# frutiemax92/YAT

Measured on AMD Instinct MI355X. Metric: images/sec (whole node) SANA-1.6B 1024px bf16 training step, higher is better.
Workload: dtype bf16; 1 GPU; train_sana.py: SANA-1.6B (D=2240, 20 blocks) 1024px, bf16, full fine-tune, cached latents/text embeds, aspect buckets [(32, 32), (16, 64), (24, 42), (44, 22)] round-robin, prompts of 20..300 tokens (text rows packed: the masked padding rows to T=512 are not computed), AdamW+clip; global_batch=8, per_gpu_batch=8, seq_len=1024, parallelism=dp1, num_layers=20, params=1604462784

## Files before the change

### yat_amd/csrc/linear_attn.hip

```cpp
#include "common.hpp"
#include "../../include/yat_hip.h"

namespace {

constexpr int C = 32;
constexpr int SS = 33 * C;
constexpr int TB = 256;

__device__ __forceinline__ bf16x8 zero8() {
    bf16x8 z;
#pragma unroll
    for (int e = 0; e < 8; ++e) z[e] = (__bf16)0.0f;
    return z;
}
__device__ __forceinline__ bf16x8 relu8(bf16x8 v) {
    u32x4 u = __builtin_bit_cast(u32x4, v);
#pragma unroll
    for (int i = 0; i < 4; ++i) {
        const uint32_t neg = (u[i] >> 15) & 0x00010001u;
        u[i] &= ~(neg * 0xffffu);
    }
    return __builtin_bit_cast(bf16x8, u);
}
__device__ __forceinline__ void split8(const float* x, bf16x8& hi, bf16x8& lo) {
#pragma unroll
    for (int e = 0; e < 8; ++e) {
        const __bf16 h = (__bf16)x[e];
        hi[e] = h;
        lo[e] = (__bf16)(x[e] - (float)h);
    }
}
__device__ __forceinline__ void state_frag_rows(const float* S, int row0, int nrows, int lane, bf16x8& hi, bf16x8& lo) {
    float x[8];
    const int r = row0 + (lane & 15);
    if (r < nrows) {
        const f32x4 a = *reinterpret_cast<const f32x4*>(S + r * C + 8 * (lane >> 4));
        const f32x4 b = *reinterpret_cast<const f32x4*>(S + r * C + 8 * (lane >> 4) + 4);
        x[0] = a[0]; x[1] = a[1]; x[2] = a[2]; x[3] = a[3]; x[4] = b[0]; x[5] = b[1]; x[6] = b[2]; x[7] = b[3];
    } else {
#pragma unroll
        for (int e = 0; e < 8; ++e) x[e] = 0.f;
    }
    split8(x, hi, lo);
}
template <bool ACC_ORDER>
__device__ __forceinline__ void state_frag_cols(const float* S, int col0, int lane, bf16x8& hi, bf16x8& lo) {
    float x[8];
    const int c = col0 + (lane & 15), g = lane >> 4;
#pragma unroll
    for (int j = 0; j < 8; ++j) {
        const int cp = ACC_ORDER ? (j < 4 ? 4 * g + j : 16 + 4 * g + (j - 4)) : 8 * g + j;
        x[j] = S[cp * C + c];
    }
    split8(x, hi, lo);
}
__device__ __forceinline__ void acc2frag_hilo(const f32x4& a, const f32x4& b, bf16x8& hi, bf16x8& lo) {
    const float x[8] = {a[0], a[1], a[2], a[3], b[0], b[1], b[2], b[3]};
    split8(x, hi, lo);
}
__device__ __forceinline__ bf16x8 tok_frag(const bf16_t* base, int ld, int tok, int N, int lane) {
    bf16x8 z = zero8();
    if (tok < N) z = *reinterpret_cast<const bf16x8*>(base + (int64_t)tok * ld + 8 * (lane >> 4));
    return z;
}
__device__ __forceinline__ u32x2 tok4_raw(const bf16_t* base, int ld, int tok, int N, int c0) {
    return tok < N ? *reinterpret_cast<const u32x2*>(base + (int64_t)tok * ld + c0) : u32x2{0u, 0u};
}
__device__ __forceinline__ void tok4(const bf16_t* base, int ld, int tok, int N, int c0, float* o) {
    if (tok < N) unpack4(*reinterpret_cast<const u32x2*>(base + (int64_t)tok * ld + c0), o);
    else { o[0] = o[1] = o[2] = o[3] = 0.f; }
}

__global__ __launch_bounds__(256) void la_state_kernel(int N, const bf16_t* qkv, int ld, int k_off, int v_off,
                                                       uint64_t bytes, float* S_out) {
    __shared__ __attribute__((aligned(16))) char lds[4 * 8192 + 4 * 6 * 64 * 16];
    const int lane = threadIdx.x & 63, wave = __builtin_amdgcn_readfirstlane(threadIdx.x >> 6);
    int h, b, unused_z;
    xcd_contiguous3(h, b, unused_z);
    char* kt = lds + wave * 8192;
    char* vt = kt + 4096;
    const __amdgpu_buffer_rsrc_t rs = make_rsrc(qkv, bytes);
    const int per = ((N + 3) / 4 + 63) / 64 * 64;
    const int n_begin = wave * per, n_end = min(N, n_begin + per);
    const int64_t head_off = (int64_t)b * N * ld + h * C;

    f32x4 acc[2][3];
#pragma unroll
    for (int i = 0; i < 2; ++i)
#pragma unroll
        for (int j = 0; j < 3; ++j) acc[i][j] = f32x4{0.f, 0.f, 0.f, 0.f};
    bf16x8 ones = zero8();
    if ((lane & 15) == 0) {
#pragma unroll
        for (int e = 0; e < 8; ++e) ones[e] = (__bf16)1.0f;
    }
    const uint32_t g = lane >> 4, q4 = (lane & 15) >> 2, p4 = lane & 3;
    for (int n0 = n_begin; n0 < n_end; n0 += 64) {
#pragma unroll
        for (int pc = 0; pc < 4; ++pc) {
            const int r = pc * 16 + (lane >> 2);
            const int slot = lane & 3;
            const int chunk = slot ^ (((r >> 3) & 1) << 1);
            const int n = n0 + r;
            const uint32_t vk = n < N ? (uint32_t)((head_off + (int64_t)n * ld + k_off + chunk * 8) * 2) : YAT_OOB;
            const uint32_t vv = n < N ? (uint32_t)((head_off + (int64_t)n * ld + v_off + chunk * 8) * 2) : YAT_OOB;
            lds_dma16(rs, (YAT_LDS void*)(kt + pc * 1024), vk);
            lds_dma16(rs, (YAT_LDS void*)(vt + pc * 1024), vv);
        }
        asm volatile("s_waitcnt vmcnt(0)" ::: "memory");
#pragma unroll
        for (int ks = 0; ks < 2; ++ks) {
            bf16x8 kf[2], vf[2];
#pragma unroll
            for (int ct = 0; ct < 2; ++ct) {
                const uint32_t col = ct * 16 + 4 * p4;
                const uint32_t r0 = ks * 32 + 8 * g + q4, r1 = r0 + 4;
                const uint32_t c0 = (col >> 3) ^ (((r0 >> 3) & 1) << 1), c1 = (col >> 3) ^ (((r1 >> 3) & 1) << 1);
                kf[ct] = relu8(cat4(lds_read_tr4(kt, r0 * 64 + c0 * 16 + (p4 & 1) * 8), lds_read_tr4(kt, r1 * 64 + c1 * 16 + (p4 & 1) * 8)));
                vf[ct] = cat4(lds_read_tr4(vt, r0 * 64 + c0 * 16 + (p4 & 1) * 8), lds_read_tr4(vt, r1 * 64 + c1 * 16 + (p4 & 1) * 8));
            }
#pragma unroll
            for (int ct = 0; ct < 2; ++ct) {
                acc[ct][0] = mfma16(kf[ct], vf[0], acc[ct][0]);
                acc[ct][1] = mfma16(kf[ct], vf[1], acc[ct][1]);
                acc[ct][2] = mfma16(kf[ct], ones, acc[ct][2]);
            }
        }
        asm volatile("s_waitcnt lgkmcnt(0)" ::: "memory");
    }
    float* red = reinterpret_cast<float*>(lds + 4 * 8192);
#pragma unroll
    for (int ct = 0; ct < 2; ++ct)
#pragma unroll
        for (int j = 0; j < 3; ++j) *reinterpret_cast<f32x4*>(red + ((wave * 6 + ct * 3 + j) * 64 + lane) * 4) = acc[ct][j];
    __syncthreads();
    if (wave == 0) {
        float* S = S_out + ((int64_t)b * gridDim.x + h) * SS;
#pragma unroll
        for (int ct = 0; ct < 2; ++ct)
#pragma unroll
            for (int j = 0; j < 3; ++j) {
                f32x4 s = f32x4{0.f, 0.f, 0.f, 0.f};
#pragma unroll
                for (int w = 0; w < 4; ++w) {
                    const f32x4 t = *reinterpret_cast<const f32x4*>(red + ((w * 6 + ct * 3 + j) * 64 + lane) * 4);
                    s[0] += t[0]; s[1] += t[1]; s[2] += t[2]; s[3] += t[3];
                }
                const int cp = j * 16 + (lane & 15);
                if (cp < 33) {
#pragma unroll
                    for (int r = 0; r < 4; ++r) S[cp * C + ct * 16 + 4 * g + r] = s[r];
                }
            }
    }
}

__device__ __forceinline__ void u_tiles(const bf16x8 (&shi)[3], const bf16x8 (&slo)[3], bf16x8 qf, f32x4 (&ut)[3]) {
#pragma unroll
    for (int t = 0; t < 3; ++t) {
        ut[t] = mfma16(shi[t], qf, f32x4{0.f, 0.f, 0.f, 0.f});
        ut[t] = mfma16(slo[t], qf, ut[t]);
    }
}

__global__ __launch_bounds__(256) void la_fwd_kernel(int N, int H, const bf16_t* qkv, int ld, const float* S_all,
                                                     bf16_t* out, int ld_out) {
    const int lane = threadIdx.x & 63, wave = threadIdx.x >> 6;
    int cx, h, b;
    xcd_contiguous3(cx, h, b);
    const float* S = S_all + ((int64_t)b * H + h) * SS;
    bf16x8 shi[3], slo[3];
#pragma unroll
    for (int t = 0; t < 3; ++t) state_frag_rows(S, t * 16, 33, lane, shi[t], slo[t]);
    const bf16_t* qb = qkv + (int64_t)b * N * ld + h * C;
    bf16_t* ob = out + (int64_t)b * N * ld_out + h * C;
    const int g = lane >> 4, li = lane & 15;
    bf16x8 qfr[4];
#pragma unroll
    for (int grp = 0; grp < 4; ++grp) qfr[grp] = tok_frag(qb, ld, cx * TB + wave * 64 + grp * 16 + li, N, lane);
#pragma unroll
    for (int grp = 0; grp < 4; ++grp) {
        const int n = cx * TB + wave * 64 + grp * 16 + li;
        f32x4 ut[3];
        u_tiles(shi, slo, relu8(qfr[grp]), ut);
        const float den = __shfl(ut[2][0], li, 64) + 1e-15f;
        const float inv = 1.0f / den;
        if (n < N) {
#pragma unroll
            for (int t = 0; t < 2; ++t)
                *reinterpret_cast<u32x2*>(ob + (int64_t)n * ld_out + t * 16 + 4 * g) =
                    pack4(ut[t][0] * inv, ut[t][1] * inv, ut[t][2] * inv, ut[t][3] * inv);
        }
    }
}

__device__ __forceinline__ uint32_t du_off(uint32_t row, uint32_t byte) {
    const uint32_t sw = (((row >> 1) & 1) | (((row >> 3) & 1) << 1)) << 1;
    return row * 128 + ((((byte >> 4) ^ sw) << 4) | (byte & 15));
}
__device__ __forceinline__ uint32_t q_off(uint32_t row, uint32_t byte) {
    return row * 64 + (byte ^ (((row >> 3) & 1) << 5));
}

__global__ __launch_bounds__(256, 3) void la_bwd_q_kernel(int N, int H, const bf16_t* qkv, int ld, const bf16_t* dout, int ld_do,
                                                       const float* S_all, bf16_t* dqkv, int ld_dq, float* dS_part) {
    __shared__ __attribute__((aligned(16))) char lds[4 * (2 * 4096 + 2048)];
    static_assert(4 * 6 * 64 * 16 <= 4 * (2 * 4096 + 2048), "reduction slab must fit in the images");
    const int lane = threadIdx.x & 63, wave = __builtin_amdgcn_readfirstlane(threadIdx.x >> 6);
    int cx, h, b;
    xcd_contiguous3(cx, h, b);
    const int g = lane >> 4, li = lane & 15, q4 = li >> 2, p4 = lane & 3;
    const float* S = S_all + ((int64_t)b * H + h) * SS;
    char* du_img = lds + wave * 10240;
    char* du_lo = du_img + 4096;
    char* q_img = du_img + 8192;
    bf16x8 shi[3], slo[3], xhi[2], xlo[2];
#pragma unroll
    for (int t = 0; t < 3; ++t) state_frag_rows(S, t * 16, 33, lane, shi[t], slo[t]);
#pragma unroll
    for (int ct = 0; ct < 2; ++ct) state_frag_cols<true>(S, ct * 16, lane, xhi[ct], xlo[ct]);
    float s32[2][4];
#pragma unroll
    for (int ct = 0; ct < 2; ++ct)
#pragma unroll
        for (int r = 0; r < 4; ++r) s32[ct][r] = S[32 * C + ct * 16 + 4 * g + r];
    const bf16_t* qb = qkv + (int64_t)b * N * ld + h * C;
    const bf16_t* dob = dout + (int64_t)b * N * ld_do + h * C;
    bf16_t* dqb = dqkv + (int64_t)b * N * ld_dq + h * C;

    f32x4 ds[3][2];
#pragma unroll
    for (int t = 0; t < 3; ++t)
#pragma unroll
        for (int ct = 0; ct < 2; ++ct) ds[t][ct] = f32x4{0.f, 0.f, 0.f, 0.f};

    bf16x8 qfr[4];
    u32x2 d4r[4][2], q4r[4][2];
#pragma unroll
    for (int s4 = 0; s4 < 4; ++s4) {
        const int n = cx * TB + wave * 64 + s4 * 16 + li;
        qfr[s4] = tok_frag(qb, ld, n, N, lane);
#pragma unroll
        for (int t = 0; t < 2; ++t) {
            d4r[s4][t] = tok4_raw(dob, ld_do, n, N, t * 16 + 4 * g);
            q4r[s4][t] = tok4_raw(qb, ld, n, N, t * 16 + 4 * g);
        }
    }
#pragma unroll
    for (int half = 0; half < 2; ++half) {
#pragma unroll
        for (int sub = 0; sub < 2; ++sub) {
            const int n0 = cx * TB + wave * 64 + half * 32 + sub * 16;
            const int n = n0 + li;
            const bf16x8 qf = relu8(qfr[half * 2 + sub]);
            f32x4 ut[3];
            u_tiles(shi, slo, qf, ut);
            const float den = __shfl(ut[2][0], li, 64) + 1e-15f;
            const float inv = 1.0f / den;
            float dot = 0.f;
            f32x4 du[2];
#pragma unroll
            for (int t = 0; t < 2; ++t) {
                float d4[4];
                unpack4(d4r[half * 2 + sub][t], d4);
#pragma unroll
                for (int r = 0; r < 4; ++r) {
                    dot += d4[r] * (ut[t][r] * inv);
                    du[t][r] = d4[r] * inv;
                }
            }
            dot += __shfl_xor(dot, 16, 64);
            dot += __shfl_xor(dot, 32, 64);
            const float du32 = -dot * inv;
            bf16x8 dhi, dlo;
            acc2frag_hilo(du[0], du[1], dhi, dlo);
            const bool valid = n < N;
#pragma unroll
            for (int ct = 0; ct < 2; ++ct) {
                f32x4 dq = mfma16(xhi[ct], dhi, f32x4{0.f, 0.f, 0.f, 0.f});
                dq = mfma16(xhi[ct], dlo, dq);
                dq = mfma16(xlo[ct], dhi, dq);
                float q4v[4];
                unpack4(q4r[half * 2 + sub][ct], q4v);
                if (valid) {
                    float o[4];
#pragma unroll
                    for (int r = 0; r < 4; ++r) o[r] = q4v[r] > 0.f ? dq[r] + s32[ct][r] * du32 : 0.f;
                    *reinterpret_cast<u32x2*>(dqb + (int64_t)n * ld_dq + ct * 16 + 4 * g) = pack4(o[0], o[1], o[2], o[3]);
                }
            }
            const int trow = sub * 16 + li;
#pragma unroll
            for (int t = 0; t < 2; ++t) {
                float hi4[4], lo4[4];
#pragma unroll
                for (int r = 0; r < 4; ++r) { hi4[r] = valid ? rbf(du[t][r]) : 0.f; lo4[r] = valid ? du[t][r] - hi4[r] : 0.f; }
                *reinterpret_cast<u32x2*>(du_img + du_off(trow, (t * 16 + 4 * g) * 2)) = pack4(hi4[0], hi4[1], hi4[2], hi4[3]);
                *reinterpret_cast<u32x2*>(du_lo + du_off(trow, (t * 16 + 4 * g) * 2)) = pack4(lo4[0], lo4[1], lo4[2], lo4[3]);
            }
            {
                const float h32 = (valid && g == 0) ? rbf(du32) : 0.f, l32 = (valid && g == 0) ? du32 - h32 : 0.f;
                *reinterpret_cast<u32x2*>(du_img + du_off(trow, (32 + 4 * g) * 2)) = pack4(h32, 0.f, 0.f, 0.f);
                *reinterpret_cast<u32x2*>(du_lo + du_off(trow, (32 + 4 * g) * 2)) = pack4(l32, 0.f, 0.f, 0.f);
            }
            *reinterpret_cast<u32x2*>(du_img + du_off(trow, (48 + 4 * g) * 2)) = u32x2{0u, 0u};
            *reinterpret_cast<u32x2*>(du_lo + du_off(trow, (48 + 4 * g) * 2)) = u32x2{0u, 0u};
            *reinterpret_cast<bf16x8*>(q_img + q_off(trow, g * 16)) = qf;
        }
        asm volatile("s_waitcnt lgkmcnt(0)" ::: "memory");
        bf16x8 af[3], al[3], bfr[2];
        const uint32_t r0 = 8 * g + q4, r1 = r0 + 4;
#pragma unroll
        for (int t = 0; t < 3; ++t) {
            const uint32_t off = (t * 16 + 4 * p4) * 2;
            af[t] = cat4(lds_read_tr4(du_img, du_off(r0, off)), lds_read_tr4(du_img, du_off(r1, off)));
            al[t] = cat4(lds_read_tr4(du_lo, du_off(r0, off)), lds_read_tr4(du_lo, du_off(r1, off)));
        }
#pragma unroll
        for (int ct = 0; ct < 2; ++ct) {
            const uint32_t off = (ct * 16 + 4 * p4) * 2;
            bfr[ct] = cat4(lds_read_tr4(q_img, q_off(r0, off)), lds_read_tr4(q_img, q_off(r1, off)));
        }
#pragma unroll
        for (int t = 0; t < 3; ++t)
#pragma unroll
            for (int ct = 0; ct < 2; ++ct) {
                ds[t][ct] = mfma16(af[t], bfr[ct], ds[t][ct]);
                ds[t][ct] = mfma16(al[t], bfr[ct], ds[t][ct]);
            }
        asm volatile("s_waitcnt lgkmcnt(0)" ::: "memory");
    }
    __syncthreads();
    float* red = reinterpret_cast<float*>(lds);
#pragma unroll
    for (int t = 0; t < 3; ++t)
#pragma unroll
        for (int ct = 0; ct < 2; ++ct) *reinterpret_cast<f32x4*>(red + ((wave * 6 + t * 2 + ct) * 64 + lane) * 4) = ds[t][ct];
    __syncthreads();
    if (wave == 0) {
        float* slab = dS_part + (((int64_t)b * H + h) * gridDim.x + cx) * SS;
#pragma unroll
        for (int t = 0; t < 3; ++t)
#pragma unroll
            for (int ct = 0; ct < 2; ++ct) {
                f32x4 s = f32x4{0.f, 0.f, 0.f, 0.f};
#pragma unroll
                for (int w = 0; w < 4; ++w) {
                    const f32x4 v = *reinterpret_cast<const f32x4*>(red + ((w * 6 + t * 2 + ct) * 64 + lane) * 4);
                    s[0] += v[0]; s[1] += v[1]; s[2] += v[2]; s[3] += v[3];
                }
#pragma unroll
                for (int r = 0; r < 4; ++r) {
                    const int cp = t * 16 + 4 * g + r;
                    if (cp < 33) slab[cp * C + ct * 16 + li] = s[r];
                }
            }
    }
}

__global__ void la_reduce_slabs_kernel(int nbh, int nchunks, const float* part, float* dS) {
    const int64_t i = (int64_t)blockIdx.x * blockDim.x + threadIdx.x;
    if (i >= (int64_t)nbh * SS) return;
    const int64_t bh = i / SS, e = i % SS;
    float s = 0.f;
    for (int c = 0; c < nchunks; ++c) s += part[(bh * nchunks + c) * SS + e];
    dS[i] = s;
}

__global__ __launch_bounds__(256) void la_bwd_kv_kernel(int N, int H, const bf16_t* qkv, int ld, int k_off, int v_off,
                                                        const float* dS_all, bf16_t* dqkv, int ld_dq) {
    const int lane = threadIdx.x & 63, wave = threadIdx.x >> 6;
    int cx, h, b;
    xcd_contiguous3(cx, h, b);
    const int g = lane >> 4, li = lane & 15;
    const float* dS = dS_all + ((int64_t)b * H + h) * SS;
    bf16x8 rhi[2], rlo[2], chi[2], clo[2];
#pragma unroll
    for (int t = 0; t < 2; ++t) state_frag_rows(dS, t * 16, 32, lane, rhi[t], rlo[t]);
#pragma unroll
    for (int ct = 0; ct < 2; ++ct) state_frag_cols<false>(dS, ct * 16, lane, chi[ct], clo[ct]);
    float s32[2][4];
#pragma unroll
    for (int ct = 0; ct < 2; ++ct)
#pragma unroll
        for (int r = 0; r < 4; ++r) s32[ct][r] = dS[32 * C + ct * 16 + 4 * g + r];
    const bf16_t* kb = qkv + (int64_t)b * N * ld + h * C + k_off;
    const bf16_t* vb = qkv + (int64_t)b * N * ld + h * C + v_off;
    bf16_t* dkb = dqkv + (int64_t)b * N * ld_dq + h * C + k_off;
    bf16_t* dvb = dqkv + (int64_t)b * N * ld_dq + h * C + v_off;
    bf16x8 kfr[4], vfr[4];
    u32x2 k4r[4][2];
#pragma unroll
    for (int grp = 0; grp < 4; ++grp) {
        const int n = cx * TB + wave * 64 + grp * 16 + li;
        kfr[grp] = tok_frag(kb, ld, n, N, lane);
        vfr[grp] = tok_frag(vb, ld, n, N, lane);
#pragma unroll
        for (int t = 0; t < 2; ++t) k4r[grp][t] = tok4_raw(kb, ld, n, N, t * 16 + 4 * g);
    }
#pragma unroll
    for (int grp = 0; grp < 4; ++grp) {
        const int n = cx * TB + wave * 64 + grp * 16 + li;
        const bf16x8 kf = relu8(kfr[grp]);
        const bf16x8 vf = vfr[grp];
#pragma unroll
        for (int t = 0; t < 2; ++t) {
            f32x4 dv = mfma16(rhi[t], kf, f32x4{0.f, 0.f, 0.f, 0.f});
            dv = mfma16(rlo[t], kf, dv);
            f32x4 dk = mfma16(chi[t], vf, f32x4{0.f, 0.f, 0.f, 0.f});
            dk = mfma16(clo[t], vf, dk);
            float k4[4];
            unpack4(k4r[grp][t], k4);
            if (n < N) {
                *reinterpret_cast<u32x2*>(dvb + (int64_t)n * ld_dq + t * 16 + 4 * g) = pack4(dv[0], dv[1], dv[2], dv[3]);
                float o[4];
#pragma unroll
                for (int r = 0; r < 4; ++r) o[r] = k4[r] > 0.f ? dk[r] + s32[t][r] : 0.f;
                *reinterpret_cast<u32x2*>(dkb + (int64_t)n * ld_dq + t * 16 + 4 * g) = pack4(o[0], o[1], o[2], o[3]);
            }
        }
    }
}

}

extern "C" {

uint64_t yat_linear_attn_workspace_bytes(int B, int N, int H) {
    const uint64_t nchunks = (N + TB - 1) / TB;
    return (uint64_t)B * H * SS * sizeof(float) * (2 + nchunks);
}

static int la_check(int B, int N, int H, int ld, int k_off, int v_off) {
    if (B <= 0 || N <= 0 || H <= 0 || (ld & 7) || (k_off & 7) || (v_off & 7)) return YAT_EINVAL;
    if ((uint64_t)B * N * ld * 2 > 0x7fffffffull) return YAT_EINVAL;
    return YAT_OK;
}

int yat_linear_attn_fwd(int B, int N, int H, const void* qkv, int ld, int k_off, int v_off, void* out, int ld_out,
                        void* workspace, yat_stream_t stream) {
    if (la_check(B, N, H, ld, k_off, v_off) || (ld_out & 7) || !qkv || !out || !workspace) return YAT_EINVAL;
    float* S = (float*)workspace;
    hipLaunchKernelGGL(la_state_kernel, dim3(H, B), dim3(256), 0, (hipStream_t)stream, N, (const bf16_t*)qkv, ld, k_off, v_off,
                       (uint64_t)B * N * ld * 2, S);
    YAT_CHECK_LAUNCH();
    hipLaunchKernelGGL(la_fwd_kernel, dim3((N + TB - 1) / TB, H, B), dim3(256), 0, (hipStream_t)stream, N, H,
                       (const bf16_t*)qkv, ld, (const float*)S, (bf16_t*)out, ld_out);
    YAT_CHECK_LAUNCH();
    return YAT_OK;
}

int yat_linear_attn_bwd(int B, int N, int H, const void* qkv, int ld, int k_off, int v_off, const void* dout, int ld_dout,
                        void* dqkv, int ld_dqkv, const float* state, void* workspace, yat_stream_t stream) {
    if (la_check(B, N, H, ld, k_off, v_off) || (ld_dout & 7) || (ld_dqkv & 7) || !qkv || !dout || !dqkv || !workspace)
        return YAT_EINVAL;
    const int nchunks = (N + TB - 1) / TB;
    float* S = (float*)workspace;
    float* dS = S + (int64_t)B * H * SS;
    float* part = dS + (int64_t)B * H * SS;
    hipStream_t st = (hipStream_t)stream;
    if (state) {
        S = const_cast<float*>(state);
    } else {
        hipLaunchKernelGGL(la_state_kernel, dim3(H, B), dim3(256), 0, st, N, (const bf16_t*)qkv, ld, k_off, v_off,
                           (uint64_t)B * N * ld * 2, S);
        YAT_CHECK_LAUNCH();
    }
    hipLaunchKernelGGL(la_bwd_q_kernel, dim3(nchunks, H, B), dim3(256), 0, st, N, H, (const bf16_t*)qkv, ld,
                       (const bf16_t*)dout, ld_dout, (const float*)S, (bf16_t*)dqkv, ld_dqkv, part);
    YAT_CHECK_LAUNCH();
    const int64_t tot = (int64_t)B * H * SS;
    hipLaunchKernelGGL(la_reduce_slabs_kernel, dim3((unsigned)((tot + 255) / 256)), dim3(256), 0, st, B * H, nchunks,
                       (const float*)part, dS);
    YAT_CHECK_LAUNCH();
    hipLaunchKernelGGL(la_bwd_kv_kernel, dim3(nchunks, H, B), dim3(256), 0, st, N, H, (const bf16_t*)qkv, ld, k_off, v_off,
                       (const float*)dS, (bf16_t*)dqkv, ld_dqkv);
    YAT_CHECK_LAUNCH();
    return YAT_OK;
}

}
```

Before: 106.0 images/s.

## Fuse slab reduction into linear-attn bwd kv and pair heads for full-line stores

```diff
diff --git a/yat_amd/csrc/linear_attn.hip b/yat_amd/csrc/linear_attn.hip
--- a/yat_amd/csrc/linear_attn.hip
+++ b/yat_amd/csrc/linear_attn.hip
@@ -30,12 +30,35 @@
         lo[e] = (__bf16)(x[e] - (float)h);
     }
 }
-__device__ __forceinline__ void state_frag_rows(const float* S, int row0, int nrows, int lane, bf16x8& hi, bf16x8& lo) {
+struct OneState {
+    const float* S;
+    __device__ __forceinline__ float at(int i) const { return S[i]; }
+    __device__ __forceinline__ f32x4 at4(int i) const { return *reinterpret_cast<const f32x4*>(S + i); }
+};
+struct SlabSum {
+    const float* part;
+    int n;
+    __device__ __forceinline__ float at(int i) const {
+        float s = 0.f;
+        for (int c = 0; c < n; ++c) s += part[(int64_t)c * SS + i];
+        return s;
+    }
+    __device__ __forceinline__ f32x4 at4(int i) const {
+        f32x4 s = f32x4{0.f, 0.f, 0.f, 0.f};
+        for (int c = 0; c < n; ++c) {
+            const f32x4 t = *reinterpret_cast<const f32x4*>(part + (int64_t)c * SS + i);
+            s[0] += t[0]; s[1] += t[1]; s[2] += t[2]; s[3] += t[3];
+        }
+        return s;
+    }
+};
+template <class St>
+__device__ __forceinline__ void state_frag_rows(const St S, int row0, int nrows, int lane, bf16x8& hi, bf16x8& lo) {
     float x[8];
     const int r = row0 + (lane & 15);
     if (r < nrows) {
-        const f32x4 a = *reinterpret_cast<const f32x4*>(S + r * C + 8 * (lane >> 4));
-        const f32x4 b = *reinterpret_cast<const f32x4*>(S + r * C + 8 * (lane >> 4) + 4);
+        const f32x4 a = S.at4(r * C + 8 * (lane >> 4));
+        const f32x4 b = S.at4(r * C + 8 * (lane >> 4) + 4);
         x[0] = a[0]; x[1] = a[1]; x[2] = a[2]; x[3] = a[3]; x[4] = b[0]; x[5] = b[1]; x[6] = b[2]; x[7] = b[3];
     } else {
 #pragma unroll
@@ -43,14 +66,14 @@
     }
     split8(x, hi, lo);
 }
-template <bool ACC_ORDER>
-__device__ __forceinline__ void state_frag_cols(const float* S, int col0, int lane, bf16x8& hi, bf16x8& lo) {
+template <bool ACC_ORDER, class St>
+__device__ __forceinline__ void state_frag_cols(const St S, int col0, int lane, bf16x8& hi, bf16x8& lo) {
     float x[8];
     const int c = col0 + (lane & 15), g = lane >> 4;
 #pragma unroll
     for (int j = 0; j < 8; ++j) {
         const int cp = ACC_ORDER ? (j < 4 ? 4 * g + j : 16 + 4 * g + (j - 4)) : 8 * g + j;
-        x[j] = S[cp * C + c];
+        x[j] = S.at(cp * C + c);
     }
     split8(x, hi, lo);
 }
@@ -163,12 +186,13 @@
     }
 }
 
-__global__ __launch_bounds__(256) void la_fwd_kernel(int N, int H, const bf16_t* qkv, int ld, const float* S_all,
+__global__ __launch_bounds__(256) void la_fwd_kernel(int N, int H, int h0, const bf16_t* qkv, int ld, const float* S_all,
                                                      bf16_t* out, int ld_out) {
     const int lane = threadIdx.x & 63, wave = threadIdx.x >> 6;
     int cx, h, b;
     xcd_contiguous3(cx, h, b);
-    const float* S = S_all + ((int64_t)b * H + h) * SS;
+    h += h0;
+    const OneState S{S_all + ((int64_t)b * H + h) * SS};
     bf16x8 shi[3], slo[3];
 #pragma unroll
     for (int t = 0; t < 3; ++t) state_frag_rows(S, t * 16, 33, lane, shi[t], slo[t]);
@@ -192,6 +216,63 @@
                     pack4(ut[t][0] * inv, ut[t][1] * inv, ut[t][2] * inv, ut[t][3] * inv);
         }
     }
+}
+
+__device__ __forceinline__ uint32_t pair_off(uint32_t row, uint32_t byte) {
+    return row * 128 + ((swz128(row, byte >> 4) << 4) | (byte & 15));
+}
+__device__ __forceinline__ void pair_store_rows(const char* img, int rows, bf16_t* dst, int ld, int n0, int N, int lane) {
+    for (int r0 = 0; r0 < rows; r0 += 8) {
+        const int r = r0 + (lane >> 3), ch = lane & 7;
+        if (n0 + r < N)
+            *reinterpret_cast<u32x4*>(dst + (int64_t)(n0 + r) * ld + ch * 8) = *reinterpret_cast<const u32x4*>(img + pair_off(r, ch * 16));
+    }
+}
+__device__ __forceinline__ uint32_t pos_mask8(bf16x8 v) {
+    uint32_t m = 0;
+#pragma unroll
+    for (int e = 0; e < 8; ++e) m |= ((float)v[e] > 0.f ? 1u : 0u) << e;
+    return m;
+}
+__device__ __forceinline__ uint32_t out_layout_mask(uint32_t m8, int li, int g) {
+    const uint32_t lo = (uint32_t)__shfl((int)m8, li + 16 * (g >> 1), 64), hi = (uint32_t)__shfl((int)m8, li + 16 * (2 + (g >> 1)), 64);
+    const int sh = 4 * (g & 1);
+    return ((lo >> sh) & 15u) | (((hi >> sh) & 15u) << 4);
+}
+
+__global__ __launch_bounds__(256) void la_fwd_pair_kernel(int N, int H, const bf16_t* qkv, int ld, const float* S_all,
+                                                          bf16_t* out, int ld_out) {
+    __shared__ __attribute__((aligned(16))) char lds[4 * 8192];
+    const int lane = threadIdx.x & 63, wave = __builtin_amdgcn_readfirstlane(threadIdx.x >> 6);
+    int cx, hp, b;
+    xcd_contiguous3(cx, hp, b);
+    const int h = 2 * hp, g = lane >> 4, li = lane & 15, n0 = cx * TB + wave * 64;
+    char* img = lds + wave * 8192;
+    const bf16_t* qb = qkv + (int64_t)b * N * ld + h * C;
+    bf16x8 qfr[2][4];
+#pragma unroll
+    for (int grp = 0; grp < 4; ++grp)
+#pragma unroll
+        for (int hh = 0; hh < 2; ++hh) qfr[hh][grp] = tok_frag(qb + hh * C, ld, n0 + grp * 16 + li, N, lane);
+#pragma unroll
+    for (int hh = 0; hh < 2; ++hh) {
+        const OneState S{S_all + ((int64_t)b * H + h + hh) * SS};
+        bf16x8 shi[3], slo[3];
+#pragma unroll
+        for (int t = 0; t < 3; ++t) state_frag_rows(S, t * 16, 33, lane, shi[t], slo[t]);
+#pragma unroll
+        for (int grp = 0; grp < 4; ++grp) {
+            f32x4 ut[3];
+            u_tiles(shi, slo, relu8(qfr[hh][grp]), ut);
+            const float den = __shfl(ut[2][0], li, 64) + 1e-15f;
+            const float inv = 1.0f / den;
+#pragma unroll
+            for (int t = 0; t < 2; ++t)
+                *reinterpret_cast<u32x2*>(img + pair_off(grp * 16 + li, hh * 64 + t * 32 + 8 * g)) =
+                    pack4(ut[t][0] * inv, ut[t][1] * inv, ut[t][2] * inv, ut[t][3] * inv);
+        }
+    }
+    pair_store_rows(img, 64, out + (int64_t)b * N * ld_out + h * C, ld_out, n0, N, lane);
 }
 
 __device__ __forceinline__ uint32_t du_off(uint32_t row, uint32_t byte) {
@@ -216,9 +297,9 @@
     char* q_img = du_img + 8192;
     bf16x8 shi[3], slo[3], xhi[2], xlo[2];
 #pragma unroll
-    for (int t = 0; t < 3; ++t) state_frag_rows(S, t * 16, 33, lane, shi[t], slo[t]);
-#pragma unroll
-    for (int ct = 0; ct < 2; ++ct) state_frag_cols<true>(S, ct * 16, lane, xhi[ct], xlo[ct]);
+    for (int t = 0; t < 3; ++t) state_frag_rows(OneState{S}, t * 16, 33, lane, shi[t], slo[t]);
+#pragma unroll
+    for (int ct = 0; ct < 2; ++ct) state_frag_cols<true>(OneState{S}, ct * 16, lane, xhi[ct], xlo[ct]);
     float s32[2][4];
 #pragma unroll
     for (int ct = 0; ct < 2; ++ct)
@@ -358,67 +439,118 @@
     }
 }
 
-__global__ void la_reduce_slabs_kernel(int nbh, int nchunks, const float* part, float* dS) {
-    const int64_t i = (int64_t)blockIdx.x * blockDim.x + threadIdx.x;
-    if (i >= (int64_t)nbh * SS) return;
-    const int64_t bh = i / SS, e = i % SS;
-    float s = 0.f;
-    for (int c = 0; c < nchunks; ++c) s += part[(bh * nchunks + c) * SS + e];
-    dS[i] = s;
-}
-
-__global__ __launch_bounds__(256) void la_bwd_kv_kernel(int N, int H, const bf16_t* qkv, int ld, int k_off, int v_off,
-                                                        const float* dS_all, bf16_t* dqkv, int ld_dq) {
+struct KvState {
+    bf16x8 rhi[2], rlo[2], chi[2], clo[2];
+    float s32[2][4];
+    __device__ __forceinline__ void load(const SlabSum dS, int lane) {
+#pragma unroll
+        for (int t = 0; t < 2; ++t) state_frag_rows(dS, t * 16, 32, lane, rhi[t], rlo[t]);
+#pragma unroll
+        for (int ct = 0; ct < 2; ++ct) state_frag_cols<false>(dS, ct * 16, lane, chi[ct], clo[ct]);
+#pragma unroll
+        for (int ct = 0; ct < 2; ++ct) {
+            const f32x4 v = dS.at4(32 * C + ct * 16 + 4 * (lane >> 4));
+            s32[ct][0] = v[0]; s32[ct][1] = v[1]; s32[ct][2] = v[2]; s32[ct][3] = v[3];
+        }
+    }
+    __device__ __forceinline__ void apply(bf16x8 kraw, bf16x8 vf, uint32_t kpos, u32x2 (&dk2)[2], u32x2 (&dv2)[2]) const {
+        const bf16x8 kf = relu8(kraw);
+#pragma unroll
+        for (int t = 0; t < 2; ++t) {
+            f32x4 dv = mfma16(rhi[t], kf, f32x4{0.f, 0.f, 0.f, 0.f});
+            dv = mfma16(rlo[t], kf, dv);
+            f32x4 dk = mfma16(chi[t], vf, f32x4{0.f, 0.f, 0.f, 0.f});
+            dk = mfma16(clo[t], vf, dk);
+            float o[4];
+#pragma unroll
+            for (int r = 0; r < 4; ++r) o[r] = ((kpos >> (4 * t + r)) & 1u) ? dk[r] + s32[t][r] : 0.f;
+            dv2[t] = pack4(dv[0], dv[1], dv[2], dv[3]);
+            dk2[t] = pack4(o[0], o[1], o[2], o[3]);
+        }
+    }
+};
+
+__global__ __launch_bounds__(256) void la_bwd_kv_kernel(int N, int H, int h0, const bf16_t* qkv, int ld, int k_off, int v_off,
+                                                        const float* part, bf16_t* dqkv, int ld_dq) {
     const int lane = threadIdx.x & 63, wave = threadIdx.x >> 6;
     int cx, h, b;
     xcd_contiguous3(cx, h, b);
+    h += h0;
     const int g = lane >> 4, li = lane & 15;
-    const float* dS = dS_all + ((int64_t)b * H + h) * SS;
-    bf16x8 rhi[2], rlo[2], chi[2], clo[2];
-#pragma unroll
-    for (int t = 0; t < 2; ++t) state_frag_rows(dS, t * 16, 32, lane, rhi[t], rlo[t]);
-#pragma unroll
-    for (int ct = 0; ct < 2; ++ct) state_frag_cols<false>(dS, ct * 16, lane, chi[ct], clo[ct]);
-    float s32[2][4];
-#pragma unroll
-    for (int ct = 0; ct < 2; ++ct)
-#pragma unroll
-        for (int r = 0; r < 4; ++r) s32[ct][r] = dS[32 * C + ct * 16 + 4 * g + r];
     const bf16_t* kb = qkv + (int64_t)b * N * ld + h * C + k_off;
     const bf16_t* vb = qkv + (int64_t)b * N * ld + h * C + v_off;
     bf16_t* dkb = dqkv + (int64_t)b * N * ld_dq + h * C + k_off;
     bf16_t* dvb = dqkv + (int64_t)b * N * ld_dq + h * C + v_off;
     bf16x8 kfr[4], vfr[4];
-    u32x2 k4r[4][2];
 #pragma unroll
     for (int grp = 0; grp < 4; ++grp) {
         const int n = cx * TB + wave * 64 + grp * 16 + li;
         kfr[grp] = tok_frag(kb, ld, n, N, lane);
         vfr[grp] = tok_frag(vb, ld, n, N, lane);
-#pragma unroll
-        for (int t = 0; t < 2; ++t) k4r[grp][t] = tok4_raw(kb, ld, n, N, t * 16 + 4 * g);
-    }
+    }
+    KvState st;
+    st.load(SlabSum{part + ((int64_t)b * H + h) * gridDim.x * SS, (int)gridDim.x}, lane);
 #pragma unroll
     for (int grp = 0; grp < 4; ++grp) {
         const int n = cx * TB + wave * 64 + grp * 16 + li;
-        const bf16x8 kf = relu8(kfr[grp]);
-        const bf16x8 vf = vfr[grp];
-#pragma unroll
-        for (int t = 0; t < 2; ++t) {
-            f32x4 dv = mfma16(rhi[t], kf, f32x4{0.f, 0.f, 0.f, 0.f});
-            dv = mfma16(rlo[t], kf, dv);
-            f32x4 dk = mfma16(chi[t], vf, f32x4{0.f, 0.f, 0.f, 0.f});
-            dk = mfma16(clo[t], vf, dk);
-            float k4[4];
-            unpack4(k4r[grp][t], k4);
-            if (n < N) {
-                *reinterpret_cast<u32x2*>(dvb + (int64_t)n * ld_dq + t * 16 + 4 * g) = pack4(dv[0], dv[1], dv[2], dv[3]);
-                float o[4];
-#pragma unroll
-                for (int r = 0; r < 4; ++r) o[r] = k4[r] > 0.f ? dk[r] + s32[t][r] : 0.f;
-                *reinterpret_cast<u32x2*>(dkb + (int64_t)n * ld_dq + t * 16 + 4 * g) = pack4(o[0], o[1], o[2], o[3]);
-            }
-        }
+        u32x2 dk2[2], dv2[2];
+        st.apply(kfr[grp], vfr[grp], out_layout_mask(pos_mask8(kfr[grp]), li, g), dk2, dv2);
+        if (n < N) {
+#pragma unroll
+            for (int t = 0; t < 2; ++t) {
+                *reinterpret_cast<u32x2*>(dvb + (int64_t)n * ld_dq + t * 16 + 4 * g) = dv2[t];
+                *reinterpret_cast<u32x2*>(dkb + (int64_t)n * ld_dq + t * 16 + 4 * g) = dk2[t];
+            }
+        }
+    }
+}
+
+constexpr int KV_ST = 16;
+__global__ __launch_bounds__(256) void la_bwd_kv_pair_kernel(int N, int H, const bf16_t* qkv, int ld, int k_off, int v_off,
+                                                             const float* part, bf16_t* dqkv, int ld_dq) {
+    constexpr int SUB = KV_ST / 16, IMG = KV_ST * 128;
+    __shared__ __attribute__((aligned(16))) char lds[2 * 2 * 2 * IMG];
+    const int lane = threadIdx.x & 63, wave = __builtin_amdgcn_readfirstlane(threadIdx.x >> 6);
+    int cx, hp, b;
+    xcd_contiguous3(cx, hp, b);
+    const int hh = wave & 1, wp = wave >> 1, h = 2 * hp + hh;
+    const int g = lane >> 4, li = lane & 15, n_base = cx * TB + wp * 128;
+    const bf16_t* kb = qkv + (int64_t)b * N * ld + h * C + k_off;
+    const bf16_t* vb = qkv + (int64_t)b * N * ld + h * C + v_off;
+    bf16_t* dst = dqkv + (int64_t)b * N * ld_dq + 2 * hp * C + (hh ? v_off : k_off);
+    bf16x8 kfr[2][SUB], vfr[2][SUB];
+#pragma unroll
+    for (int sub = 0; sub < SUB; ++sub) {
+        kfr[0][sub] = tok_frag(kb, ld, n_base + sub * 16 + li, N, lane);
+        vfr[0][sub] = tok_frag(vb, ld, n_base + sub * 16 + li, N, lane);
+    }
+    KvState st;
+    st.load(SlabSum{part + ((int64_t)b * H + h) * gridDim.x * SS, (int)gridDim.x}, lane);
+#pragma unroll
+    for (int s = 0; s < 128 / KV_ST; ++s) {
+        const int n0 = n_base + s * KV_ST;
+        if (s + 1 < 128 / KV_ST) {
+#pragma unroll
+            for (int sub = 0; sub < SUB; ++sub) {
+                kfr[(s + 1) & 1][sub] = tok_frag(kb, ld, n0 + KV_ST + sub * 16 + li, N, lane);
+                vfr[(s + 1) & 1][sub] = tok_frag(vb, ld, n0 + KV_ST + sub * 16 + li, N, lane);
+            }
+        }
+        char* buf = lds + (wp * 2 + (s & 1)) * 2 * IMG;
+        if (n0 < N) {
+#pragma unroll
+            for (int sub = 0; sub < SUB; ++sub) {
+                u32x2 dk2[2], dv2[2];
+                st.apply(kfr[s & 1][sub], vfr[s & 1][sub], out_layout_mask(pos_mask8(kfr[s & 1][sub]), li, g), dk2, dv2);
+#pragma unroll
+                for (int t = 0; t < 2; ++t) {
+                    *reinterpret_cast<u32x2*>(buf + pair_off(sub * 16 + li, hh * 64 + t * 32 + 8 * g)) = dk2[t];
+                    *reinterpret_cast<u32x2*>(buf + IMG + pair_off(sub * 16 + li, hh * 64 + t * 32 + 8 * g)) = dv2[t];
+                }
+            }
+        }
+        __syncthreads();
+        pair_store_rows(buf + hh * IMG, KV_ST, dst, ld_dq, n0, N, lane);
     }
 }
 
@@ -437,16 +569,28 @@
     return YAT_OK;
 }
 
+static bool la_line_ok(const void* p, int ld) { return ((uintptr_t)p & 127) == 0 && (ld & 63) == 0; }
+
 int yat_linear_attn_fwd(int B, int N, int H, const void* qkv, int ld, int k_off, int v_off, void* out, int ld_out,
                         void* workspace, yat_stream_t stream) {
     if (la_check(B, N, H, ld, k_off, v_off) || (ld_out & 7) || !qkv || !out || !workspace) return YAT_EINVAL;
     float* S = (float*)workspace;
-    hipLaunchKernelGGL(la_state_kernel, dim3(H, B), dim3(256), 0, (hipStream_t)stream, N, (const bf16_t*)qkv, ld, k_off, v_off,
+    const int nchunks = (N + TB - 1) / TB;
+    hipStream_t st = (hipStream_t)stream;
+    hipLaunchKernelGGL(la_state_kernel, dim3(H, B), dim3(256), 0, st, N, (const bf16_t*)qkv, ld, k_off, v_off,
                        (uint64_t)B * N * ld * 2, S);
     YAT_CHECK_LAUNCH();
-    hipLaunchKernelGGL(la_fwd_kernel, dim3((N + TB - 1) / TB, H, B), dim3(256), 0, (hipStream_t)stream, N, H,
-                       (const bf16_t*)qkv, ld, (const float*)S, (bf16_t*)out, ld_out);
-    YAT_CHECK_LAUNCH();
+    const int hpair = la_line_ok(qkv, ld) && la_line_ok(out, ld_out) ? H / 2 : 0;
+    if (hpair) {
+        hipLaunchKernelGGL(la_fwd_pair_kernel, dim3(nchunks, hpair, B), dim3(256), 0, st, N, H, (const bf16_t*)qkv, ld,
+                           (const float*)S, (bf16_t*)out, ld_out);
+        YAT_CHECK_LAUNCH();
+    }
+    if (H > 2 * hpair) {
+        hipLaunchKernelGGL(la_fwd_kernel, dim3(nchunks, H - 2 * hpair, B), dim3(256), 0, st, N, H, 2 * hpair, (const bf16_t*)qkv, ld,
+                           (const float*)S, (bf16_t*)out, ld_out);
+        YAT_CHECK_LAUNCH();
+    }
     return YAT_OK;
 }
 
@@ -469,13 +613,17 @@
     hipLaunchKernelGGL(la_bwd_q_kernel, dim3(nchunks, H, B), dim3(256), 0, st, N, H, (const bf16_t*)qkv, ld,
                        (const bf16_t*)dout, ld_dout, (const float*)S, (bf16_t*)dqkv, ld_dqkv, part);
     YAT_CHECK_LAUNCH();
-    const int64_t tot = (int64_t)B * H * SS;
-    hipLaunchKernelGGL(la_reduce_slabs_kernel, dim3((unsigned)((tot + 255) / 256)), dim3(256), 0, st, B * H, nchunks,
-                       (const float*)part, dS);
-    YAT_CHECK_LAUNCH();
-    hipLaunchKernelGGL(la_bwd_kv_kernel, dim3(nchunks, H, B), dim3(256), 0, st, N, H, (const bf16_t*)qkv, ld, k_off, v_off,
-                       (const float*)dS, (bf16_t*)dqkv, ld_dqkv);
-    YAT_CHECK_LAUNCH();
+    const int hpair = la_line_ok(qkv, ld) && la_line_ok(dqkv, ld_dqkv) && !(k_off & 63) && !(v_off & 63) ? H / 2 : 0;
+    if (hpair) {
+        hipLaunchKernelGGL(la_bwd_kv_pair_kernel, dim3(nchunks, hpair, B), dim3(256), 0, st, N, H, (const bf16_t*)qkv, ld, k_off,
+                           v_off, (const float*)part, (bf16_t*)dqkv, ld_dqkv);
+        YAT_CHECK_LAUNCH();
+    }
+    if (H > 2 * hpair) {
+        hipLaunchKernelGGL(la_bwd_kv_kernel, dim3(nchunks, H - 2 * hpair, B), dim3(256), 0, st, N, H, 2 * hpair, (const bf16_t*)qkv,
+                           ld, k_off, v_off, (const float*)part, (bf16_t*)dqkv, ld_dqkv);
+        YAT_CHECK_LAUNCH();
+    }
     return YAT_OK;
 }
 
```

Result: no change. 105.8 images/s (-0.2%).
